# smileyenot983/reconstructor

Hardware: AMD Instinct MI355X
Metric: descriptor pair-distances/s + BA LM-iterations/s (1k cams, 100k pts) (higher is better)
Workload: dtype f16+f64

## Files before the change

reconstructor_amd/csrc/match.hip:

```cpp
#include "rcn_internal.h"

#include <algorithm>
#include <cmath>

typedef _Float16 half8 __attribute__((ext_vector_type(8)));
typedef float f32x16 __attribute__((ext_vector_type(16)));
typedef float f32x4 __attribute__((ext_vector_type(4)));
typedef unsigned u32x4 __attribute__((ext_vector_type(4)));

#define RCN_QT 512
#define RCN_GROUP 4
#define RCN_TBL_BYTES ((RCN_GROUP * 24 + 127) / 128 * 128)
#define RCN_NBUF 4
#define RCN_PD 2
#define RCN_CHUNK_ROWS (1ll << 27)
#define RCN_BT 64
#define RCN_PAD_HN 1.0e30f
#define RCN_I8_IDX_BITS 12
#define RCN_I8_IDX_MASK ((1u << RCN_I8_IDX_BITS) - 1u)
#define RCN_I8_PAD_ACC ((1 << (32 - RCN_I8_IDX_BITS)) - 1)
#define RCN_I8_BT 128
#define RCN_I8_RES_MAX 8.01
#define RCN_I8_M_MAX 720.0
#define RCN_I8_PEAK_MAX 8.0
// ... 635 lines not shown
        }
    } else {
        for (int k = 0; k < D; ++k) {
            double d = (double)q[k] - (double)t[k];
            acc = fma(d, d, acc);
        }
    }
    return acc;
}

__device__ __forceinline__ bool ratio_pass(double d2_best, double d2_second, float ratio)
{
    float dist0 = sqrtf((float)d2_best);
    float dist1 = sqrtf((float)d2_second);
    return dist0 < ratio * dist1;
}

struct RerankArgs {
    const ImgDev *imgs;
    const int32_t *pairs;
    const uint2 *cand;
    int32_t *out;
    int64_t out_stride;
    unsigned long long *fb_list;
    unsigned *fb_count;
    unsigned *fb_tacc;
    unsigned long long *sv_list;
    unsigned *sv_count;
    int32_t n_pairs, kq_stride, D, qblocks, pair_base;
    uint32_t idx_mask;
    float ratio;
    const ScaleDev *sc;
    int32_t all_to_fallback;
    int32_t filter_pass, rerank_pass;
};

#ifdef RCN_DIAG
#define RCN_FILTER_PASS(a) ((a).filter_pass != 0)
#define RCN_RERANK_PASS(a) ((a).rerank_pass != 0)
#else
#define RCN_FILTER_PASS(a) false
#define RCN_RERANK_PASS(a) false
#endif

__device__ __forceinline__ int certify(double ea, int ia, double eb, double lbnc, float ratio)
{
    const bool nn_certain = ea < lbnc;
    double lb1 = fmin(eb, lbnc), lb0 = fmin(ea, lbnc);
    if (lb1 < 0.0) lb1 = 0.0;
    if (lb0 < 0.0) lb0 = 0.0;
    if (nn_certain && ratio_pass(ea, lb1, ratio)) return ia;
    if (!ratio_pass(lb0, eb, ratio)) return -1;
    return -2;
}

__device__ __forceinline__ double coarse_eps(const ScaleDev &a, double nq2)
{
    const double nq = sqrt(nq2) * (1.0 + 1e-12);
    const double mag = a.s2 * nq * a.n_max;
    return a.c_in * nq * a.n_max + a.c_sub * (nq + a.n_max) + 1e-9 + a.c_acc * (a.hn_max + mag) +
           6.0e-8 * a.hn_max;
}
__device__ __forceinline__ double acc_to_d2(const ScaleDev &a, double nq2, double acc)
{
    return nq2 + (2.0 / a.s2) * (acc - a.bias);
}

__device__ __forceinline__ double key_lo(const ScaleDev &S, unsigned k, uint32_t mask)
{
    return S.coarse_i8 ? (double)(k >> RCN_I8_IDX_BITS) : (double)__uint_as_float(k & ~mask);
}
__device__ __forceinline__ double key_hi(const ScaleDev &S, unsigned k, uint32_t mask)
{
    return S.coarse_i8 ? (double)(k >> RCN_I8_IDX_BITS) : (double)__uint_as_float((k & ~mask) + mask + 1u);
}
__device__ __forceinline__ bool key_is_pad(const ScaleDev &S, unsigned k, uint32_t mask)
{
    return S.coarse_i8 ? (k >> RCN_I8_IDX_BITS) >= (unsigned)RCN_I8_PAD_ACC : !(__uint_as_float(k & ~mask) < 1.0e29f);
}
__device__ __forceinline__ int key_idx(const ScaleDev &S, unsigned k, uint32_t mask)
{
    return (int)(k & (S.coarse_i8 ? RCN_I8_IDX_MASK : mask));
}
__device__ __forceinline__ double coarse_eps_row(const ScaleDev &S, const ImgDev &qi, int q, double nq2)
{
    if (!S.coarse_i8) return coarse_eps(S, nq2);
    const float2 n = qi.i8n[q];
    return ((double)n.x * S.rho + (double)n.y * (S.tau + S.rho)) * (1.0 + 1e-9) + 0.5 + 1.0e-3;
}

__device__ __forceinline__ double big_lower_bound(const unsigned long long *bigmin, double nq2)
{
    const double b2 = __longlong_as_double((long long)*bigmin);
    if (!(b2 <= 1.7976931348623157e308)) return b2;
    const double d = sqrt(b2) * (1.0 - 1e-12) - sqrt(nq2) * (1.0 + 1e-12);
    return d > 0.0 ? d * d * (1.0 - 1e-9) : 0.0;
}

__device__ __forceinline__ unsigned mid_thr_acc(const ScaleDev &S, const ImgDev &qi, int q, double nq2, double eb, unsigned key2, uint32_t mask)
{
    if (!S.coarse_i8 || key_is_pad(S, key2, mask) || !(fabs(eb) <= 1.7976931348623157e308)) return 0u;
    const double d2 = eb * (1.0 + S.rel_slack) + S.rel_slack * (nq2 + S.n_max * S.n_max);
    const double v = floor(S.bias + S.hs2 * (d2 - nq2) + coarse_eps_row(S, qi, q, nq2)) + 1.0;
    if (!(v >= 1.0) || v >= (double)RCN_I8_PAD_ACC) return 0u;
    return (unsigned)v;
}

__device__ __forceinline__ void list_append(unsigned long long *list, unsigned *count, bool want,
                                            unsigned long long entry, unsigned *side = nullptr, unsigned side_value = 0u)
{
    const unsigned long long m = __ballot(want);
    if (!m) return;
    const int lane = threadIdx.x & 63;
    const int leader = __ffsll((long long)m) - 1;
    unsigned base = 0;
    if (lane == leader) base = atomicAdd(count, (unsigned)__popcll(m));
    base = __shfl(base, leader);
    if (want) {
        const unsigned slot = base + __popcll(m & ((1ull << lane) - 1ull));
        list[slot] = entry;
        if (side) side[slot] = side_value;
    }
}

#define RCN_FT 1024
#define RCN_FR 4
#define RCN_FB (RCN_FT * RCN_FR)
__global__ __launch_bounds__(RCN_FT) void k_filter(RerankArgs a)
{
    __shared__ unsigned wcnt[2][RCN_FT / 64];
    __shared__ unsigned wbase[2][RCN_FT / 64];
    const int pl = blockIdx.x / a.qblocks, pair = a.pair_base + pl;
    const int q0 = (blockIdx.x - pl * a.qblocks) * RCN_FB + threadIdx.x;
    const ScaleDev S = *a.sc;
    const ImgDev qi = a.imgs[a.pairs[2 * pair]];
    const ImgDev ti = a.imgs[a.pairs[2 * pair + 1]];
    unsigned survm = 0u, fbm = 0u;
    double nq2v[RCN_FR];
    uint2 cv[RCN_FR];
#pragma unroll
    for (int r = 0; r < RCN_FR; ++r) {
        const int q = q0 + r * RCN_FT;
        nq2v[r] = 0.0; cv[r] = make_uint2(0u, 0u);
        if (q < qi.K && ti.K >= 2) {
            nq2v[r] = qi.nrm2[q];
            if (!a.all_to_fallback) cv[r] = a.cand[(size_t)pair * a.kq_stride + q];
        }
    }
#pragma unroll
    for (int r = 0; r < RCN_FR; ++r) {
        const int q = q0 + r * RCN_FT;
        bool surv = false, fb = false;
        if (q < qi.K) {
            int32_t res = -1;
            if (ti.K >= 2) {
                const double nq2 = nq2v[r];
                const uint2 c = cv[r];
                if (a.all_to_fallback || !(nq2 < S.thr2)  || key_is_pad(S, c.y, a.idx_mask)) fb = true;
                else {
                    const double eps = coarse_eps_row(S, qi, q, nq2);
                    const double lb_big = big_lower_bound(ti.bigmin, nq2);
                    const double slack = S.rel_slack * (nq2 + S.n_max * S.n_max);
                    const double lo = key_lo(S, c.x, a.idx_mask);
                    const double hi = key_hi(S, c.y, a.idx_mask);
                    double lb0 = fmin(acc_to_d2(S, nq2, lo - eps) - slack, lb_big);
                    const double ub1 = acc_to_d2(S, nq2, hi + eps) + slack;
                    if (lb0 < 0.0) lb0 = 0.0;
                    surv = ratio_pass(lb0, ub1, a.ratio) || RCN_FILTER_PASS(a);
                    if (surv && ti.K > 2 && !RCN_FILTER_PASS(a)) {
                        const double hi0 = key_hi(S, c.x, a.idx_mask);
                        const double lo1 = key_lo(S, c.y, a.idx_mask);
                        const double ub0 = acc_to_d2(S, nq2, hi0 + eps) + slack;
                        double lbnc = fmin(acc_to_d2(S, nq2, lo1 - eps) - slack, lb_big);
                        if (lbnc < 0.0) lbnc = 0.0;
                        if (ub0 >= 0.0 && ub0 < lbnc && ratio_pass(ub0, lbnc, a.ratio)) {
                            res = (int32_t)key_idx(S, c.x, a.idx_mask);
                            surv = false;
                        }
                    }
                }
            }
            a.out[(size_t)pair * a.out_stride + q] = res;
        }
        survm |= surv ? 1u << r : 0u;
        fbm |= fb ? 1u << r : 0u;
    }
    const int lane = threadIdx.x & 63, w = threadIdx.x >> 6, nw = blockDim.x >> 6;
    unsigned ns = 0, nf = 0;
#pragma unroll
    for (int r = 0; r < RCN_FR; ++r) { ns += (unsigned)__popcll(__ballot(survm >> r & 1u)); nf += (unsigned)__popcll(__ballot(fbm >> r & 1u)); }
    if (lane == 0) { wcnt[0][w] = ns; wcnt[1][w] = nf; }
    __syncthreads();
    if (threadIdx.x < 2) {
        unsigned tot = 0;
        for (int i = 0; i < nw; ++i) { wbase[threadIdx.x][i] = tot; tot += wcnt[threadIdx.x][i]; }
        const unsigned base = tot ? atomicAdd(threadIdx.x == 0 ? a.sv_count : a.fb_count, tot) : 0u;
        for (int i = 0; i < nw; ++i) wbase[threadIdx.x][i] += base;
    }
    __syncthreads();
    const unsigned long long lt = (1ull << lane) - 1ull;
    unsigned bs = wbase[0][w], bf = wbase[1][w];
#pragma unroll
    for (int r = 0; r < RCN_FR; ++r) {
        const unsigned long long entry = ((unsigned long long)pair << 32) | (unsigned)(q0 + r * RCN_FT);
        const unsigned long long ms = __ballot(survm >> r & 1u), mf = __ballot(fbm >> r & 1u);
        if (survm >> r & 1u) a.sv_list[bs + __popcll(ms & lt)] = entry;
        if (fbm >> r & 1u) a.fb_list[bf + __popcll(mf & lt)] = entry;
        bs += (unsigned)__popcll(ms); bf += (unsigned)__popcll(mf);
    }
}

#define RR_ROWS 192
#define RR_LD 36
__global__ __launch_bounds__(64) void k_rerank_lds(RerankArgs a)
{
    __shared__ __attribute__((aligned(16))) float tile[RR_ROWS * RR_LD];
    __shared__ const float *rowptr[RR_ROWS];
    const int lane = threadIdx.x;
    const unsigned n = *a.sv_count;
    const int D = a.D;
    const int nchunk = (D + 31) / 32;
    const ScaleDev S = *a.sc;
    for (unsigned g = blockIdx.x; g * 64u < n; g += gridDim.x) {
        const unsigned sidx = g * 64u + lane;
        const bool live = sidx < n;
        const unsigned long long e = a.sv_list[live ? sidx : g * 64u];
        const int pair = (int)(e >> 32), q = (int)(e & 0xFFFFFFFFu);
        const ImgDev qi = a.imgs[a.pairs[2 * pair]];
        const ImgDev ti = a.imgs[a.pairs[2 * pair + 1]];
        const uint2 c = a.cand[(size_t)pair * a.kq_stride + q];
        int ia = key_idx(S, c.x, a.idx_mask), ib = key_idx(S, c.y, a.idx_mask);
        if (ib >= ti.K) ib = ia;
        __syncthreads();
        rowptr[lane] = qi.f32 + (size_t)q * D;
        rowptr[64 + lane] = ti.f32 + (size_t)ia * D;
        rowptr[128 + lane] = ti.f32 + (size_t)ib * D;
        __syncthreads();
        double acc = 0.0, acc2 = 0.0;
        const float *qrow = tile + lane * RR_LD;
        const float *trow = tile + (64 + lane) * RR_LD;
        const float *trow2 = tile + (128 + lane) * RR_LD;
        for (int ch = 0; ch < nchunk; ++ch) {
            const int col = ch * 32 + (lane & 7) * 4;
#pragma unroll
            for (int i = 0; i < RR_ROWS / 8; ++i) {
                const int r = i * 8 + (lane >> 3);
                float4 v = make_float4(0.f, 0.f, 0.f, 0.f);
                if (col < D) v = *reinterpret_cast<const float4 *>(rowptr[r] + col);
                *reinterpret_cast<float4 *>(tile + r * RR_LD + (lane & 7) * 4) = v;
            }
            __syncthreads();
            const int kmax = min(32, D - ch * 32);
            for (int k4 = 0; k4 < kmax; k4 += 4) {
                const float4 x = *reinterpret_cast<const float4 *>(qrow + k4);
                const float4 y = *reinterpret_cast<const float4 *>(trow + k4);
                const float4 z = *reinterpret_cast<const float4 *>(trow2 + k4);
                double d;
                d = (double)x.x - (double)y.x; acc = fma(d, d, acc);
                d = (double)x.y - (double)y.y; acc = fma(d, d, acc);
                d = (double)x.z - (double)y.z; acc = fma(d, d, acc);
                d = (double)x.w - (double)y.w; acc = fma(d, d, acc);
                d = (double)x.x - (double)z.x; acc2 = fma(d, d, acc2);
                d = (double)x.y - (double)z.y; acc2 = fma(d, d, acc2);
                d = (double)x.z - (double)z.z; acc2 = fma(d, d, acc2);
                d = (double)x.w - (double)z.w; acc2 = fma(d, d, acc2);
            }
            __syncthreads();
        }
        bool fb = false;
        unsigned tacc = 0u;
        if (live) {
            double ea = acc, eb = acc2;
            if (ib != ia && (eb < ea || (eb == ea && ib < ia))) { ea = acc2; eb = acc; const int t = ia; ia = ib; ib = t; }
            int res = -2;
            if (ti.K > 2 && ib != ia) {
                const double nq2 = qi.nrm2[q];
                const double lbacc = key_lo(S, c.y, a.idx_mask);
                const double lbnc = fmin(acc_to_d2(S, nq2, lbacc - coarse_eps_row(S, qi, q, nq2)) - S.rel_slack * (nq2 + S.n_max * S.n_max), big_lower_bound(ti.bigmin, nq2));
                res = RCN_RERANK_PASS(a) ? -2 : certify(ea, ia, eb, lbnc, a.ratio);
                if (res == -2 && a.fb_tacc) tacc = mid_thr_acc(S, qi, q, nq2, eb, c.y, a.idx_mask);
            }
            if (res >= 0) a.out[(size_t)pair * a.out_stride + q] = res;
            else if (res == -2) fb = true;
        }
        list_append(a.fb_list, a.fb_count, fb, e, a.fb_tacc, tacc);
    }
}

__global__ void k_rerank_generic(RerankArgs a)
{
    const unsigned n = *a.sv_count;
    const ScaleDev S = *a.sc;
    for (unsigned s = blockIdx.x * blockDim.x + threadIdx.x; s < n; s += gridDim.x * blockDim.x) {
        const unsigned long long e = a.sv_list[s];
        const int pair = (int)(e >> 32), q = (int)(e & 0xFFFFFFFFu);
        const ImgDev qi = a.imgs[a.pairs[2 * pair]];
        const ImgDev ti = a.imgs[a.pairs[2 * pair + 1]];
        const uint2 c = a.cand[(size_t)pair * a.kq_stride + q];
        int ia = key_idx(S, c.x, a.idx_mask), ib = key_idx(S, c.y, a.idx_mask);
        const float *qrow = qi.f32 + (size_t)q * a.D;
        double ea = exact_d2<false>(qrow, ti.f32 + (size_t)ia * a.D, a.D);
        double eb = exact_d2<false>(qrow, ti.f32 + (size_t)ib * a.D, a.D);
        if (eb < ea || (eb == ea && ib < ia)) { double te = ea; ea = eb; eb = te; ia = ib; }
        double lbnc = INFINITY;
        const double nq2 = qi.nrm2[q];
        if (ti.K > 2) {
            const double lbacc = key_lo(S, c.y, a.idx_mask);
            lbnc = fmin(acc_to_d2(S, nq2, lbacc - coarse_eps_row(S, qi, q, nq2)) - S.rel_slack * (nq2 + S.n_max * S.n_max), big_lower_bound(ti.bigmin, nq2));
        }
        int res = RCN_RERANK_PASS(a) ? -2 : certify(ea, ia, eb, lbnc, a.ratio);
        if (res == -2) {
            unsigned slot = atomicAdd(a.fb_count, 1u);
            a.fb_list[slot] = e;
            if (a.fb_tacc) a.fb_tacc[slot] = ti.K > 2 && ib != ia ? mid_thr_acc(S, qi, q, nq2, eb, c.y, a.idx_mask) : 0u;
            res = -1;
        }
        a.out[(size_t)pair * a.out_stride + q] = res;
    }
}

__device__ __forceinline__ void merge_top2(double &b0, int &i0, double &b1, int &i1, double c0, int j0, double c1, int j1)
{
    const bool mine = (b0 < c0) || (b0 == c0 && i0 < j0);
    const double f0 = mine ? b0 : c0; const int fi0 = mine ? i0 : j0;
    const double l0 = mine ? c0 : b0; const int li0 = mine ? j0 : i0;
    const double s0 = mine ? b1 : c1; const int si0 = mine ? i1 : j1;
    const bool pick = (l0 < s0) || (l0 == s0 && li0 < si0);
    b0 = f0; i0 = fi0;
    b1 = pick ? l0 : s0; i1 = pick ? li0 : si0;
}

template <bool VEC4>
__global__ __launch_bounds__(256) void k_exact_rows(const ImgDev *__restrict__ imgs,
                                                     const int32_t *__restrict__ pairs,
                                                     const unsigned long long *__restrict__ list,
                                                     const unsigned *__restrict__ count, int D,
                                                     float ratio, int32_t *__restrict__ out,
                                                     int64_t out_stride, unsigned skip = 0)
{
    __shared__ double sb[4][2];
    __shared__ int si[4][2];
    const int lane = threadIdx.x & 63, w = threadIdx.x >> 6;
    const unsigned n = *count;
    for (unsigned it = skip + blockIdx.x; it < n; it += gridDim.x) {
        const unsigned long long e = list[it];
        const int pair = (int)(e >> 32), q = (int)(e & 0xFFFFFFFFu);
        const ImgDev qi = imgs[pairs[2 * pair]];
        const ImgDev ti = imgs[pairs[2 * pair + 1]];
        const float *qrow = qi.f32 + (size_t)q * D;
        double b0 = INFINITY, b1 = INFINITY;
        int i0 = 0x7FFFFFFF, i1 = 0x7FFFFFFF;
        for (int j = threadIdx.x; j < ti.K; j += 256) {
            double d = exact_d2<VEC4>(qrow, ti.f32 + (size_t)j * D, D);
            if (d < b0) { b1 = b0; i1 = i0; b0 = d; i0 = j; }
            else if (d < b1) { b1 = d; i1 = j; }
        }
        for (int o = 32; o; o >>= 1) {
            const double c0 = __shfl_xor(b0, o), c1 = __shfl_xor(b1, o);
            const int j0 = __shfl_xor(i0, o), j1 = __shfl_xor(i1, o);
            merge_top2(b0, i0, b1, i1, c0, j0, c1, j1);
        }
        __syncthreads();
        if (lane == 0) { sb[w][0] = b0; sb[w][1] = b1; si[w][0] = i0; si[w][1] = i1; }
        __syncthreads();
        if (threadIdx.x == 0) {
            for (int k = 1; k < 4; ++k) merge_top2(b0, i0, b1, i1, sb[k][0], si[k][0], sb[k][1], si[k][1]);
            out[(size_t)pair * out_stride + q] = ratio_pass(b0, b1, ratio) ? i0 : -1;
        }
    }
// ... 323 lines not shown
                }
            }
        }
    }
}
__global__ __launch_bounds__(256, 4) void k_mid_eval(MidArgs a)
{
    __shared__ __attribute__((aligned(16))) float tt[256 * MID_LD];
    __shared__ __attribute__((aligned(16))) float tq[RCN_MIDQ * MID_LD];
    __shared__ const float *qptr[RCN_MIDQ];
    __shared__ float thr[RCN_MIDQ], qnorm[RCN_MIDQ];
    __shared__ float red[4][RCN_MIDQ][2];
    __shared__ unsigned qslot[RCN_MIDQ];
    __shared__ int s_need2, s_bin, s_nown;
    const int t = threadIdx.x, lane = t & 63, w = t >> 6;
    const unsigned n_items = *a.n_items;
    for (unsigned it = blockIdx.x; it < n_items; it += gridDim.x) {
        __syncthreads();
        if (t == 0) {
            int lo = 0, hi = a.n_slots;
            while (hi - lo > 1) { const int mid = (lo + hi) >> 1; if (a.ibase[mid] <= it) lo = mid; else hi = mid; }
            s_bin = lo;
            s_need2 = 0;
        }
        __syncthreads();
        const int bin = s_bin;
        const unsigned k = it - a.ibase[bin], h = a.offs[bin + 1] - a.offs[bin];
        const int first = (int)(a.offs[bin] + RCN_MIDQ * k), nall = (int)min((unsigned)RCN_MIDQ, h - RCN_MIDQ * k);
        const ImgDev ti = a.imgs[bin];
        if (t < 64) {
            const bool own = t < nall && a.tacc[first + t] == 0u;
            const unsigned long long om = __ballot(own);
            if (t == 0) s_nown = __popcll(om);
            if (own) {
                const int o = __popcll(om & ((1ull << t) - 1ull));
                const unsigned long long e = a.sorted[first + t];
                const int pair = (int)(e >> 32), q = (int)(e & 0xFFFFFFFFu);
                const ImgDev qi = a.imgs[a.pairs[2 * pair]];
                qslot[o] = (unsigned)(first + t);
                qptr[o] = qi.f32 + (size_t)q * a.D;
                qnorm[o] = (float)(sqrt(qi.nrm2[q]) * (1.0 + 1e-6));
                const float th = a.thr[first + t];
                thr[o] = th;
                if (!(th < INFINITY)) s_need2 = 1;
            }
        }
        __syncthreads();
        const int nq = s_nown;
        if (nq == 0) continue;
        float m1[RCN_MIDQ], m2[RCN_MIDQ];
        if (!s_need2) {
            mid_sweep<0>(a, ti, qptr, nq, qslot, thr, qnorm, ti.K, tt, tq, m1, m2);
            continue;
        }
        const int prefix = min(ti.K, max(512, ti.K / 4));
#pragma unroll
        for (int q = 0; q < RCN_MIDQ; ++q) { m1[q] = INFINITY; m2[q] = INFINITY; }
        mid_sweep<1>(a, ti, qptr, nq, qslot, thr, qnorm, prefix, tt, tq, m1, m2);
#pragma unroll
        for (int q = 0; q < RCN_MIDQ; ++q) {
            float b1 = m1[q], b2 = m2[q];
            for (int o = 32; o; o >>= 1) {
                const float c1 = __shfl_xor(b1, o), c2 = __shfl_xor(b2, o);
                const float lo = fminf(b1, c1), hi = fmaxf(b1, c1);
                b2 = fminf(hi, fminf(b2, c2)); b1 = lo;
            }
            if (lane == 0) { red[w][q][0] = b1; red[w][q][1] = b2; }
        }
        __syncthreads();
        if (t < nq) {
            float b1 = red[0][t][0], b2 = red[0][t][1];
            for (int kk = 1; kk < 4; ++kk) {
                const float c1 = red[kk][t][0], c2 = red[kk][t][1];
                const float lo = fminf(b1, c1), hi = fmaxf(b1, c1);
                b2 = fminf(hi, fminf(b2, c2)); b1 = lo;
            }
            thr[t] = b2 < INFINITY ? b2 + fabsf(b2) * 1.0e-6f : INFINITY;
        }
        __syncthreads();
        mid_sweep<2>(a, ti, qptr, nq, qslot, thr, qnorm, ti.K, tt, tq, m1, m2);
    }
}
#include "mid_i8.h"
__global__ __launch_bounds__(256) void k_mid_exact(MidArgs a)
{
    const unsigned n = mid_rows(a);
    const int lane = threadIdx.x & 63;
    for (unsigned r = blockIdx.x * 4 + (threadIdx.x >> 6); r < n; r += gridDim.x * 4) {
        const unsigned long long e = a.sorted[r];
        const int pair = (int)(e >> 32), q = (int)(e & 0xFFFFFFFFu);
        const unsigned cnt = a.ccount[r];
        if (cnt > (unsigned)RCN_MIDCAP) {
            if (lane == 0) a.fb2_list[atomicAdd(a.fb2_count, 1u)] = e;
            continue;
        }
        const ImgDev qi = a.imgs[a.pairs[2 * pair]];
        const ImgDev ti = a.imgs[a.pairs[2 * pair + 1]];
        double b0 = INFINITY, b1 = INFINITY;
        int i0 = 0x7FFFFFFF, i1 = 0x7FFFFFFF;
        if (lane < (int)cnt) {
            i0 = a.clist[(size_t)r * RCN_MIDCAP + lane];
            b0 = exact_d2<true>(qi.f32 + (size_t)q * a.D, ti.f32 + (size_t)i0 * a.D, a.D);
            if (!(b0 < INFINITY)) { b0 = INFINITY; i0 = 0x7FFFFFFF; }
        }
        for (int o = 32; o; o >>= 1) {
            const double c0 = __shfl_xor(b0, o), c1 = __shfl_xor(b1, o);
            const int j0 = __shfl_xor(i0, o), j1 = __shfl_xor(i1, o);
            merge_top2(b0, i0, b1, i1, c0, j0, c1, j1);
        }
        if (lane == 0) a.out[(size_t)pair * a.out_stride + q] = ratio_pass(b0, b1, a.ratio) ? i0 : -1;
    }
}

__global__ void k_unique_claim(const ImgDev *__restrict__ imgs, const int32_t *__restrict__ pairs,
                               const int32_t *__restrict__ out, int64_t out_stride,
                               int32_t *__restrict__ owner, int owner_stride, int qblocks, int pair_base)
{
    const int pl = blockIdx.x / qblocks, pair = pair_base + pl;
    const int q = (blockIdx.x - pl * qblocks) * blockDim.x + threadIdx.x;
    if (q >= imgs[pairs[2 * pair]].K) return;
    const int t = out[(size_t)pair * out_stride + q];
    if (t >= 0) atomicMin(owner + (size_t)pair * owner_stride + t, q);
}

__global__ void k_unique_emit(const ImgDev *__restrict__ imgs, const int32_t *__restrict__ pairs,
                              int32_t *__restrict__ out, int64_t out_stride,
                              const int32_t *__restrict__ owner, int owner_stride,
                              int32_t *__restrict__ counts, int qblocks, int pair_base)
{
    const int pl = blockIdx.x / qblocks, pair = pair_base + pl;
    const int q = (blockIdx.x - pl * qblocks) * blockDim.x + threadIdx.x;
    if (q >= out_stride) return;
    int32_t *o = out + (size_t)pair * out_stride + q;
    bool keep = false;
    if (q < imgs[pairs[2 * pair]].K) {
        const int t = *o;
        keep = t >= 0 && owner[(size_t)pair * owner_stride + t] == q;
    }
    if (!keep) *o = -1;
    const unsigned long long m = __ballot(keep);
    if ((threadIdx.x & 63) == 0 && m) atomicAdd(counts + pair, (int)__popcll(m));
}

#define RCN_UNIQ_LDS 8192
__global__ __launch_bounds__(256) void k_unique_pair(const ImgDev *__restrict__ imgs, const int32_t *__restrict__ pairs,
                                                     int32_t *__restrict__ out, int64_t out_stride,
                                                     int32_t *__restrict__ counts, int pair_base)
{
    __shared__ int owner[RCN_UNIQ_LDS];
    __shared__ int wsum[4];
    const int pair = pair_base + blockIdx.x, t = threadIdx.x;
    const int Kq = imgs[pairs[2 * pair]].K, Kt = imgs[pairs[2 * pair + 1]].K;
    for (int i = t; i < Kt; i += 256) owner[i] = 0x7fffffff;
    __syncthreads();
    int32_t *row = out + (size_t)pair * out_stride;
    for (int q = t; q < Kq; q += 256) {
        const int tr = row[q];
        if (tr >= 0) atomicMin(&owner[tr], q);
    }
    __syncthreads();
    int kept = 0;
    for (int q0 = 0; q0 < out_stride; q0 += 256) {
        const int q = q0 + t;
        bool keep = false;
        if (q < out_stride) {
            const int tr = q < Kq ? row[q] : -1;
            keep = tr >= 0 && owner[tr] == q;
            if (!keep && (q >= Kq || tr >= 0)) row[q] = -1;
        }
        kept += (int)__popcll(__ballot(keep));
    }
    if ((t & 63) == 0) wsum[t >> 6] = kept;
    __syncthreads();
    if (t == 0) counts[pair] = wsum[0] + wsum[1] + wsum[2] + wsum[3];
}

__global__ void k_stats_acc(unsigned *c, int mid, unsigned midrows)
{
    if (threadIdx.x != 0 || blockIdx.x != 0) return;
    c[4] += c[0];
    c[5] += c[1];
    c[6] += mid ? c[2] + (c[0] > midrows ? c[0] - midrows : 0u) : c[0];
}

static int pad_dim(int D)
{
    if (D <= 32) return 32;
    if (D <= 64) return 64;
    if (D <= 128) return 128;
    if (D <= 256) return 256;
    return 0;
}

static hipError_t launch_rowstats(rcn_ctx *ctx, const float *x, int rows, int D, double *nrm2, unsigned *cnt)
{
    ctx->hist_rows += rows;
    unsigned long long *mx = reinterpret_cast<unsigned long long *>(cnt + 2);
    if (D % 4 == 0 && (reinterpret_cast<uintptr_t>(x) & 15) == 0)
        k_rowstats<true><<<std::max(1, std::min((rows + 15) / 16, 4096)), 256, 0, ctx->stream>>>(x, rows, D, nrm2, cnt, mx, cnt + RCN_HIST_WORD);
    else
        k_rowstats<false><<<std::max(1, std::min((rows + 3) / 4, 4096)), 256, 0, ctx->stream>>>(x, rows, D, nrm2, cnt, mx, cnt + RCN_HIST_WORD);
    return hipGetLastError();
}

static void free_image(ImgHost &im)
{
    if (im.slab >= 0) return;
    if (im.f32) (void)hipFree(im.f32);
    if (im.f16) (void)hipFree(im.f16);
    if (im.hn) (void)hipFree(im.hn);
    if (im.nrm2) (void)hipFree(im.nrm2);
    if (im.bigmin) (void)hipFree(im.bigmin);
    if (im.i8n) (void)hipFree(im.i8n);
    im.f32 = nullptr; im.f16 = nullptr; im.hn = nullptr; im.nrm2 = nullptr; im.bigmin = nullptr; im.i8n = nullptr;
}

static void free_slab(Slab &sl)
{
    if (sl.f16) (void)hipFree(sl.f16);
    if (sl.hn) (void)hipFree(sl.hn);
    if (sl.nrm2) (void)hipFree(sl.nrm2);
    if (sl.bigmin) (void)hipFree(sl.bigmin);
    if (sl.i8n) (void)hipFree(sl.i8n);
    if (sl.own_f32) (void)hipFree(sl.own_f32);
    if (sl.own_Ks) (void)hipFree(sl.own_Ks);
    sl = Slab();
}

static void retire_unreferenced_slabs(rcn_ctx *ctx)
{
    std::vector<char> used(ctx->slabs.size(), 0);
    for (const auto &kv : ctx->images)
        if (kv.second.slab >= 0) used[kv.second.slab] = 1;
    for (size_t i = 0; i < ctx->slabs.size(); ++i)
        if (ctx->slabs[i].live && !used[i]) free_slab(ctx->slabs[i]);
}

int rcn_match_release(rcn_ctx *ctx)
{
    for (auto &kv : ctx->images) free_image(kv.second);
    ctx->images.clear();
    for (Slab &sl : ctx->slabs) free_slab(sl);
    ctx->slabs.clear();
    ctx->table_host.clear();
    ctx->prepared = false;
    ctx->D = ctx->DP = 0;
    return RCN_OK;
}

static int ensure_counters(rcn_ctx *ctx)
{
    if (!ctx->counters.p) {
        RCN_HIP(ctx->counters.reserve(RCN_COUNTER_BYTES));
        RCN_HIP(hipMemsetAsync(ctx->counters.p, 0, RCN_COUNTER_BYTES, ctx->stream));
    }
    return RCN_OK;
}

static int drop_scratch_if_alone(rcn_ctx *ctx, int32_t D)
{
    if (ctx->images.empty() || ctx->D == D) return RCN_OK;
    for (const auto &kv : ctx->images)
        if (kv.first != INT32_MIN && kv.first != INT32_MIN + 1) return RCN_OK;
    RCN_HIP(hipStreamSynchronize(ctx->stream));
    for (auto &kv : ctx->images) free_image(kv.second);
    ctx->images.clear();
    ctx->prepared = false;
    return RCN_OK;
}

static int upload_common(rcn_ctx *ctx, int32_t img_id, const float *src, bool src_is_device,
                         int32_t K, int32_t D)
{
    if (!ctx || K < 0 || D <= 0 || (K > 0 && !src)) {
// ... 582 lines not shown
        if (mfma) {
            CoarseArgs ca;
            ca.imgs = imgs; ca.pairs = pairs; ca.cand = cand_c;
            const int ng_c = chunk_ng[c];
            ca.groups = ctx->groups_dev.as<int2>() + chunk_off[c];
            ca.n_groups = ng_c; ca.tiles_per_pair = tiles; ca.kq_stride = kq_stride;
            const int64_t items = (int64_t)ng_c * tiles;
            ca.items_per_xcd = (int)((items + 7) / 8);
            ca.idx_mask = idx_mask;
            ca.sc = ctx->scale_dev.as<ScaleDev>();
            const int blocks = ca.items_per_xcd * 8;
            hipError_t e;
            if (ctx->coarse_w4 && ctx->DP >= 64) {
                switch (ctx->DP) {
                case 64: e = launch_coarse_w4<64>(ctx, ca, blocks); break;
                case 128: e = launch_coarse_w4<128>(ctx, ca, blocks); break;
                default: e = launch_coarse_w4<256>(ctx, ca, blocks); break;
                }
            } else {
                const int shape = ctx->coarse_shape >= 0 ? ctx->coarse_shape : (ctx->DP == 256 ? 1 : 0);
                if (shape == 1) {
                    switch (ctx->DP) {
                    case 32: e = launch_coarse<32, 0, 1>(ctx, ca, blocks); break;
                    case 64: e = launch_coarse<64, 0, 1>(ctx, ca, blocks); break;
                    case 128: e = launch_coarse<128, 0, 1>(ctx, ca, blocks); break;
                    default:
#ifdef RCN_DIAG
                        switch (ctx->ablate) {
                        case 1: e = launch_coarse<256, 1, 1>(ctx, ca, blocks); break;
                        case 9: e = launch_coarse<256, 9, 1>(ctx, ca, blocks); break;
                        default: e = launch_coarse<256, 0, 1>(ctx, ca, blocks); break;
                        }
#else
                        e = launch_coarse<256, 0, 1>(ctx, ca, blocks);
#endif
                        break;
                    }
                } else {
                    switch (ctx->DP) {
                    case 32:
#ifdef RCN_DIAG
                        if (ctx->ablate == 1) { e = launch_coarse<32, 1, 0>(ctx, ca, blocks); break; }
                        if (ctx->ablate == 2) { e = launch_coarse<32, 2, 0>(ctx, ca, blocks); break; }
                        if (ctx->ablate == 6) { e = launch_coarse<32, 6, 0>(ctx, ca, blocks); break; }
#endif
                        e = launch_coarse<32>(ctx, ca, blocks); break;
                    case 64: e = launch_coarse<64>(ctx, ca, blocks); break;
                    case 128:
#ifdef RCN_DIAG
                        if (ctx->ablate == 1) { e = launch_coarse<128, 1, 0>(ctx, ca, blocks); break; }
                        if (ctx->ablate == 2) { e = launch_coarse<128, 2, 0>(ctx, ca, blocks); break; }
                        if (ctx->ablate == 6) { e = launch_coarse<128, 6, 0>(ctx, ca, blocks); break; }
#endif
                        e = launch_coarse<128>(ctx, ca, blocks); break;
                    default: e = launch_coarse<256>(ctx, ca, blocks); break;
                    }
                }
            }
            RCN_HIP(e);
            if (ctx->i8_allowed) {
#ifdef RCN_DIAG
                if (ctx->coarse_i8_shape == 0) e = launch_coarse_i8<0, 0>(ctx, ca, blocks);
                else if (ctx->ablate == 1) e = launch_coarse_i8<1, 1>(ctx, ca, blocks);
                else
#endif
                e = launch_coarse_i8<0, 1>(ctx, ca, blocks);
                RCN_HIP(e);
            }
        }
        if (tm) RCN_HIP(hipEventRecord(ctx->ev_c[evi][c][1], st));
        ra.cand = cand_c;
        ra.pair_base = p0;
        ra.fb_list = ctx->fb_list.as<unsigned long long>(); ra.fb_count = ccnt;
        ra.sv_list = ctx->sv_list.as<unsigned long long>(); ra.sv_count = ccnt + 1;
        if (c > 0) RCN_HIP(hipMemsetAsync(ccnt, 0, 4 * sizeof(unsigned), st));
        if (kq_max > 0) {
            const int qblocks = (kq_max + 255) / 256;
            dim3 g((unsigned)qblocks * (unsigned)np_c);
            ra.qblocks = (kq_max + RCN_FB - 1) / RCN_FB;
            k_filter<<<(unsigned)ra.qblocks * (unsigned)np_c, RCN_FT, 0, st>>>(ra);
            RCN_HIP(hipGetLastError());
            if (ctx->f32_ready) RCN_HIP(hipStreamWaitEvent(st, ctx->f32_ready, 0));
            if (mfma) {
                if (vec4) k_rerank_lds<<<ctx->prop.multiProcessorCount * 16, 64, 0, st>>>(ra);
                else k_rerank_generic<<<ctx->prop.multiProcessorCount * 8, 256, 0, st>>>(ra);
                RCN_HIP(hipGetLastError());
            }
            const int fb_blocks = ctx->prop.multiProcessorCount * 8;
            const unsigned long long *brute = ra.fb_list;
            const unsigned *brute_n = ccnt;
            if (mid) {
                char *mw = ctx->mid_ws.as<char>();
                MidArgs ma;
                memset(&ma, 0, sizeof(ma));
                ma.imgs = imgs; ma.pairs = pairs; ma.cand = cand_c; ma.fb_list = ra.fb_list; ma.fb_count = ccnt; ma.tacc_in = ra.fb_tacc;
                if (defer) {
                    MidArgs md = ma;
                    md.sc = ra.sc; md.kq_stride = kq_stride; md.D = ctx->D; md.all_to_fallback = ra.all_to_fallback; md.idx_mask = idx_mask;
                    k_mid_defer<<<ctx->prop.multiProcessorCount * 2, 256, 0, st>>>(md, (unsigned long long *)(mw + mo_def), (float *)(mw + mo_defthr), (unsigned *)(mw + mo_deftacc), ccnt, (unsigned)mid_rows_cap);
                    k_mid_defer_commit<<<1, 64, 0, st>>>(ccnt, (unsigned)mid_rows_cap);
                }
                ma.sorted = (unsigned long long *)(mw + mo_sorted); ma.thr = (float *)(mw + mo_thr); ma.ccount = (unsigned *)(mw + mo_cc); ma.tacc = (unsigned *)(mw + mo_tacc);
                ma.clist = (int32_t *)(mw + mo_cl); ma.fb2_list = (unsigned long long *)(mw + mo_fb2);
                ma.hist = (unsigned *)(mw + mo_bins); ma.offs = ma.hist + (n_slots + 1); ma.cursor = ma.offs + (n_slots + 1); ma.ibase = ma.cursor + (n_slots + 1);
                ma.n_items = ccnt + 3; ma.fb2_count = ccnt + 2;
                ma.out = out_dev; ma.out_stride = out_stride; ma.sc = ra.sc; ma.n_slots = n_slots; ma.kq_stride = kq_stride; ma.D = ctx->D;
                ma.all_to_fallback = ra.all_to_fallback; ma.idx_mask = idx_mask; ma.ratio = ratio; ma.midrows = (uint32_t)ctx->mid_rows;
                const int mb = ctx->prop.multiProcessorCount * 4;
                k_mid_hist<<<mb, 256, 0, st>>>(ma);
                k_mid_bins<<<1, 1024, 0, st>>>(ma);
                k_mid_scatter<<<mb, 256, 0, st>>>(ma);
                k_mid_eval<<<ctx->prop.multiProcessorCount * 4, 256, 0, st>>>(ma);
                if (mid_i8) k_mid_eval_i8<<<mid_i8_grid, 256, 0, st>>>(ma);
                k_mid_exact<<<mb, 256, 0, st>>>(ma);
                RCN_HIP(hipGetLastError());
                if (vec4) k_exact_rows_lds<<<fb_blocks, 64 * EX_WAVES, 0, st>>>(imgs, pairs, ma.fb2_list, ma.fb2_count, ctx->D, ratio, out_dev, out_stride);
                RCN_HIP(hipGetLastError());
                if (cap_rows > ctx->mid_rows) k_exact_rows_lds<<<fb_blocks, 64 * EX_WAVES, 0, st>>>(imgs, pairs, brute, brute_n, ctx->D, ratio, out_dev, out_stride, (unsigned)ctx->mid_rows);
            } else if (vec4) k_exact_rows_lds<<<fb_blocks, 64 * EX_WAVES, 0, st>>>(imgs, pairs, brute, brute_n, ctx->D, ratio, out_dev, out_stride);
            else k_exact_rows<false><<<fb_blocks, 256, 0, st>>>(imgs, pairs, brute, brute_n, ctx->D, ratio, out_dev, out_stride);
            RCN_HIP(hipGetLastError());
            k_stats_acc<<<1, 64, 0, st>>>(ccnt, mid ? 1 : 0, (unsigned)ctx->mid_rows);
            if (tm) RCN_HIP(hipEventRecord(ctx->ev_c[evi][c][2], st));
            if (!uniq_lds) k_unique_claim<<<g, 256, 0, st>>>(imgs, pairs, out_dev, out_stride, ctx->owner.as<int32_t>(), owner_stride, qblocks, p0);
            RCN_HIP(hipGetLastError());
        }
        if (defer) {  }
        else if (uniq_lds) k_unique_pair<<<np_c, 256, 0, st>>>(imgs, pairs, out_dev, out_stride, counts_dev, p0);
        else {
            const int eblocks = (int)((out_stride + 255) / 256);
            dim3 g((unsigned)eblocks * (unsigned)np_c);
            k_unique_emit<<<g, 256, 0, st>>>(imgs, pairs, out_dev, out_stride, ctx->owner.as<int32_t>(), owner_stride, counts_dev, eblocks, p0);
        }
        RCN_HIP(hipGetLastError());
        if (tm) RCN_HIP(hipEventRecord(ctx->ev_c[evi][c][kq_max > 0 ? 3 : 2], st));
        if (tm && kq_max <= 0) RCN_HIP(hipEventRecord(ctx->ev_c[evi][c][3], st));
    }
    ctx->ev_tail_on[evi] = false;
    if (defer) {
        if (prof) { RCN_HIP(hipEventRecord(ctx->ev_tail[evi][0], st)); ctx->ev_tail_on[evi] = true; }
        char *mw = ctx->mid_ws.as<char>();
        RCN_HIP(hipMemsetAsync(ccnt + 2, 0, 2 * sizeof(unsigned), st));
        MidArgs ma;
        memset(&ma, 0, sizeof(ma));
        ma.imgs = imgs; ma.pairs = pairs; ma.cand = nullptr; ma.fb_list = (const unsigned long long *)(mw + mo_def); ma.fb_count = ccnt + 7;
        ma.thr_in = (const float *)(mw + mo_defthr);
        ma.tacc_in = mid_i8 ? (const unsigned *)(mw + mo_deftacc) : nullptr;
        ma.sorted = (unsigned long long *)(mw + mo_sorted); ma.thr = (float *)(mw + mo_thr); ma.ccount = (unsigned *)(mw + mo_cc); ma.tacc = (unsigned *)(mw + mo_tacc);
        ma.clist = (int32_t *)(mw + mo_cl); ma.fb2_list = (unsigned long long *)(mw + mo_fb2);
        ma.hist = (unsigned *)(mw + mo_bins); ma.offs = ma.hist + (n_slots + 1); ma.cursor = ma.offs + (n_slots + 1); ma.ibase = ma.cursor + (n_slots + 1);
        ma.n_items = ccnt + 3; ma.fb2_count = ccnt + 2;
        ma.out = out_dev; ma.out_stride = out_stride; ma.sc = ra.sc; ma.n_slots = n_slots; ma.kq_stride = kq_stride; ma.D = ctx->D;
        ma.all_to_fallback = ra.all_to_fallback; ma.idx_mask = idx_mask; ma.ratio = ratio; ma.midrows = (uint32_t)mid_rows_cap;
        const int mb = ctx->prop.multiProcessorCount * 4;
        k_mid_hist<<<mb, 256, 0, st>>>(ma);
        k_mid_bins<<<1, 1024, 0, st>>>(ma);
        k_mid_scatter<<<mb, 256, 0, st>>>(ma);
        k_mid_eval<<<ctx->prop.multiProcessorCount * 4, 256, 0, st>>>(ma);
        if (mid_i8) k_mid_eval_i8<<<mid_i8_grid, 256, 0, st>>>(ma);
        k_mid_exact<<<mb, 256, 0, st>>>(ma);
        k_exact_rows_lds<<<ctx->prop.multiProcessorCount * 8, 64 * EX_WAVES, 0, st>>>(imgs, pairs, ma.fb2_list, ma.fb2_count, ctx->D, ratio, out_dev, out_stride);
        k_stats_acc_deferred<<<1, 64, 0, st>>>(ccnt);
        RCN_HIP(hipGetLastError());
        if (prof) RCN_HIP(hipEventRecord(ctx->ev_tail[evi][1], st));
        k_unique_pair<<<n_pairs, 256, 0, st>>>(imgs, pairs, out_dev, out_stride, counts_dev, 0);
        RCN_HIP(hipGetLastError());
        if (prof) RCN_HIP(hipEventRecord(ctx->ev_tail[evi][2], st));
    }
    if (prof) ctx->ev_n++;
    ctx->last_chunks = n_chunks;
    ctx->last_kq_stride = kq_stride; ctx->last_idx_mask = idx_mask; ctx->last_n_pairs = n_pairs;
    ctx->last_stats.rows_total = rows;
    ctx->last_stats.pair_distances = pd;
    ctx->last_stats.used_mfma_path = mfma ? 1 : 0;
    ctx->last_stats.coarse_dtype = mfma ? -1 : 0;
    ctx->last_stats.rows_exact_fallback = -1;
    ctx->last_stats.err_bound_d2 = -1.0;
    return RCN_OK;
}

extern "C" {

int rcn_desc_upload(rcn_ctx *ctx, int32_t img_id, const float *desc_host, int32_t K, int32_t D)
{
    if (!ctx) return RCN_ERR_ARG;
    std::lock_guard<std::mutex> lk(ctx->mu);
    return upload_common(ctx, img_id, desc_host, false, K, D);
}

int rcn_desc_upload_device(rcn_ctx *ctx, int32_t img_id, const float *desc_dev, int32_t K, int32_t D)
{
    if (!ctx) return RCN_ERR_ARG;
    std::lock_guard<std::mutex> lk(ctx->mu);
    return upload_common(ctx, img_id, desc_dev, true, K, D);
}

int rcn_desc_upload_batch_device(rcn_ctx *ctx, int32_t first_img_id, int32_t n_images,
                                 const float *desc_dev, int32_t K, int32_t D)
{
    if (!ctx) return RCN_ERR_ARG;
    std::lock_guard<std::mutex> lk(ctx->mu);
    return upload_batch(ctx, first_img_id, n_images, desc_dev, K, D);
}

int rcn_desc_upload_batch(rcn_ctx *ctx, int32_t first_img_id, int32_t n_images, const float *const *rows_host,
                          const int32_t *K, int32_t D)
{
    if (!ctx) return RCN_ERR_ARG;
    std::lock_guard<std::mutex> lk(ctx->mu);
    return upload_batch_host(ctx, first_img_id, n_images, rows_host, K, D);
}

int rcn_desc_remove(rcn_ctx *ctx, int32_t img_id)
{
    if (!ctx) return RCN_ERR_ARG;
    std::lock_guard<std::mutex> lk(ctx->mu);
    auto it = ctx->images.find(img_id);
    if (it == ctx->images.end()) return RCN_OK;
    RCN_HIP(hipSetDevice(ctx->device));
    RCN_HIP(hipStreamSynchronize(ctx->stream));
    free_image(it->second);
    ctx->images.erase(it);
    retire_unreferenced_slabs(ctx);
    ctx->prepared = false;
    if (ctx->images.empty()) ctx->D = ctx->DP = 0;
    return RCN_OK;
}

int rcn_desc_clear(rcn_ctx *ctx)
{
    if (!ctx) return RCN_ERR_ARG;
    std::lock_guard<std::mutex> lk(ctx->mu);
    RCN_HIP(hipSetDevice(ctx->device));
    RCN_HIP(hipStreamSynchronize(ctx->stream));
    rcn_match_release(ctx);
    if (ctx->counters.p) RCN_HIP(hipMemsetAsync(ctx->counters.p, 0, RCN_COUNTER_BYTES, ctx->stream));
    ctx->hist_rows = 0;
    return RCN_OK;
}

int rcn_desc_count(const rcn_ctx *ctx)
{
    if (!ctx) return 0;
// ... 271 lines not shown
```

Baseline: 4638 billion.

## Rework rerank and mid-exact kernels around a shared register-prefetched full-row LDS gather

Adds a common gather helper that loads up to 24 whole descriptor rows per wave into registers, then stores them into an XOR-swizzled LDS tile. The rerank kernel now processes 8 survivors per iteration and prefetches the next tile's rows and metadata while computing the current one. Fallback-list appends are buffered in shared memory and flushed in batches instead of using one atomic per wave per step. The mid-exact stage gets a new single-wave kernel that packs 4 query rows and 20 candidate rows per tile, and the old 256-thread kernel is kept for D above 256. Grid sizes now come from an occupancy query. The cost is fewer rows per wave, which may reduce parallelism, and higher register pressure from the 24 float4 prefetch registers.

Result: faster. 4725 billion, median of 6 (+1.9%).

```diff
diff --git a/reconstructor_amd/csrc/exact_gather.h b/reconstructor_amd/csrc/exact_gather.h
--- /dev/null
+++ b/reconstructor_amd/csrc/exact_gather.h
@@ -0,0 +1,79 @@
+#pragma once
+
+#define XG_ROWS 24
+#define XG_ROWF 256
+#define XG_TILEF (XG_ROWS * XG_ROWF)
+
+__device__ __forceinline__ unsigned xg_issue(float4 (&v)[XG_ROWS], const float *ptr, int D)
+{
+    const int col = (threadIdx.x & 63) * 4;
+    const unsigned long long pv = reinterpret_cast<unsigned long long>(ptr);
+    const int lo = (int)(unsigned)pv, hi = (int)(unsigned)(pv >> 32);
+#pragma unroll
+    for (int i = 0; i < XG_ROWS; ++i) {
+        const unsigned long long p = ((unsigned long long)(unsigned)__builtin_amdgcn_readlane(hi, i) << 32) | (unsigned)__builtin_amdgcn_readlane(lo, i);
+        v[i] = make_float4(0.f, 0.f, 0.f, 0.f);
+        if (p && col < D) v[i] = *reinterpret_cast<const float4 *>(reinterpret_cast<const float *>(p) + col);
+    }
+    return (unsigned)__ballot(ptr != nullptr) & ((1u << XG_ROWS) - 1u);
+}
+
+__device__ __forceinline__ void xg_store(float *tile, const float4 (&v)[XG_ROWS], unsigned rows)
+{
+    const int lane = threadIdx.x & 63;
+#pragma unroll
+    for (int i = 0; i < XG_ROWS; ++i)
+        if (rows >> i & 1u) *reinterpret_cast<float4 *>(tile + i * XG_ROWF + ((lane ^ (i & 15)) << 2)) = v[i];
+}
+
+__device__ __forceinline__ double xg_chain(const float *tile, int xr, int yr, int D)
+{
+    const float *x = tile + xr * XG_ROWF, *y = tile + yr * XG_ROWF;
+    const int sx = xr & 15, sy = yr & 15;
+    double acc = 0.0;
+#pragma unroll 4
+    for (int c = 0; c < D / 4; ++c) {
+        const float4 a = *reinterpret_cast<const float4 *>(x + ((c ^ sx) << 2));
+        const float4 b = *reinterpret_cast<const float4 *>(y + ((c ^ sy) << 2));
+        double d;
+        d = (double)a.x - (double)b.x; acc = fma(d, d, acc);
+        d = (double)a.y - (double)b.y; acc = fma(d, d, acc);
+        d = (double)a.z - (double)b.z; acc = fma(d, d, acc);
+        d = (double)a.w - (double)b.w; acc = fma(d, d, acc);
+    }
+    return acc;
+}
+
+#define XG_PEND 64
+#define XG_PEND_FLUSH (XG_PEND - XG_ROWS)
+struct XgPend {
+    unsigned long long e[XG_PEND];
+    unsigned side[XG_PEND];
+};
+__device__ __forceinline__ void xg_pend_flush(XgPend &p, unsigned &np, unsigned long long *list, unsigned *count, unsigned *side)
+{
+    if (!np) return;
+    const int lane = threadIdx.x & 63;
+    unsigned base = 0;
+    if (lane == 0) base = atomicAdd(count, np);
+    base = __builtin_amdgcn_readfirstlane(base);
+    if ((unsigned)lane < np) {
+        list[base + lane] = p.e[lane];
+        if (side) side[base + lane] = p.side[lane];
+    }
+    np = 0;
+}
+__device__ __forceinline__ void xg_pend_add(XgPend &p, unsigned &np, bool want, unsigned long long entry, unsigned side_value,
+                                            unsigned long long *list, unsigned *count, unsigned *side)
+{
+    const unsigned long long m = __ballot(want);
+    if (!m) return;
+    const int lane = threadIdx.x & 63;
+    if (want) {
+        const unsigned slot = np + __popcll(m & ((1ull << lane) - 1ull));
+        p.e[slot] = entry;
+        p.side[slot] = side_value;
+    }
+    np += (unsigned)__popcll(m);
+    if (np > XG_PEND_FLUSH) xg_pend_flush(p, np, list, count, side);
+}
diff --git a/reconstructor_amd/csrc/match.hip b/reconstructor_amd/csrc/match.hip
--- a/reconstructor_amd/csrc/match.hip
+++ b/reconstructor_amd/csrc/match.hip
@@ -741,28 +741,38 @@
 {
     return (int)(k & (S.coarse_i8 ? RCN_I8_IDX_MASK : mask));
 }
+__device__ __forceinline__ double coarse_eps_i8n(const ScaleDev &S, float2 n, double nq2)
+{
+    if (!S.coarse_i8) return coarse_eps(S, nq2);
+    return ((double)n.x * S.rho + (double)n.y * (S.tau + S.rho)) * (1.0 + 1e-9) + 0.5 + 1.0e-3;
+}
 __device__ __forceinline__ double coarse_eps_row(const ScaleDev &S, const ImgDev &qi, int q, double nq2)
 {
     if (!S.coarse_i8) return coarse_eps(S, nq2);
-    const float2 n = qi.i8n[q];
-    return ((double)n.x * S.rho + (double)n.y * (S.tau + S.rho)) * (1.0 + 1e-9) + 0.5 + 1.0e-3;
-}
-
-__device__ __forceinline__ double big_lower_bound(const unsigned long long *bigmin, double nq2)
-{
-    const double b2 = __longlong_as_double((long long)*bigmin);
+    return coarse_eps_i8n(S, qi.i8n[q], nq2);
+}
+
+__device__ __forceinline__ double big_lower_bound_bits(unsigned long long bigmin_bits, double nq2)
+{
+    const double b2 = __longlong_as_double((long long)bigmin_bits);
     if (!(b2 <= 1.7976931348623157e308)) return b2;
     const double d = sqrt(b2) * (1.0 - 1e-12) - sqrt(nq2) * (1.0 + 1e-12);
     return d > 0.0 ? d * d * (1.0 - 1e-9) : 0.0;
 }
-
-__device__ __forceinline__ unsigned mid_thr_acc(const ScaleDev &S, const ImgDev &qi, int q, double nq2, double eb, unsigned key2, uint32_t mask)
+__device__ __forceinline__ double big_lower_bound(const unsigned long long *bigmin, double nq2) { return big_lower_bound_bits(*bigmin, nq2); }
+
+__device__ __forceinline__ unsigned mid_thr_acc_eps(const ScaleDev &S, double eps, double nq2, double eb, unsigned key2, uint32_t mask)
 {
     if (!S.coarse_i8 || key_is_pad(S, key2, mask) || !(fabs(eb) <= 1.7976931348623157e308)) return 0u;
     const double d2 = eb * (1.0 + S.rel_slack) + S.rel_slack * (nq2 + S.n_max * S.n_max);
-    const double v = floor(S.bias + S.hs2 * (d2 - nq2) + coarse_eps_row(S, qi, q, nq2)) + 1.0;
+    const double v = floor(S.bias + S.hs2 * (d2 - nq2) + eps) + 1.0;
     if (!(v >= 1.0) || v >= (double)RCN_I8_PAD_ACC) return 0u;
     return (unsigned)v;
+}
+__device__ __forceinline__ unsigned mid_thr_acc(const ScaleDev &S, const ImgDev &qi, int q, double nq2, double eb, unsigned key2, uint32_t mask)
+{
+    if (!S.coarse_i8) return 0u;
+    return mid_thr_acc_eps(S, coarse_eps_row(S, qi, q, nq2), nq2, eb, key2, mask);
 }
 
 __device__ __forceinline__ void list_append(unsigned long long *list, unsigned *count, bool want,
@@ -869,81 +879,90 @@
     }
 }
 
-#define RR_ROWS 192
-#define RR_LD 36
+#include "exact_gather.h"
+#define RR_B (XG_ROWS / 3)
+struct RrRows {
+    unsigned long long e;
+    uint2 c;
+    const float *ptr;
+    double nq2;
+    float2 i8n;
+    unsigned long long bigmin;
+    int32_t ia, ib, tK;
+};
+__device__ __forceinline__ RrRows rr_rows(const RerankArgs &a, const ScaleDev &S, unsigned g, unsigned n)
+{
+    RrRows m;
+    const int lane = threadIdx.x & 63;
+    const unsigned sidx = g * RR_B + (lane % RR_B);
+    const bool live = sidx < n && lane < XG_ROWS;
+    m.e = a.sv_list[live ? sidx : g * RR_B];
+    const int pair = (int)(m.e >> 32), q = (int)(m.e & 0xFFFFFFFFu);
+    const ImgDev &qi = a.imgs[a.pairs[2 * pair]], &ti = a.imgs[a.pairs[2 * pair + 1]];
+    m.c = a.cand[(size_t)pair * a.kq_stride + q];
+    const float *qf = qi.f32, *tf = ti.f32;
+    m.tK = ti.K;
+    m.ia = key_idx(S, m.c.x, a.idx_mask); m.ib = key_idx(S, m.c.y, a.idx_mask);
+    if (m.ib >= m.tK) m.ib = m.ia;
+    const int role = lane / RR_B;
+    m.ptr = !live ? nullptr : role == 0 ? qf + (size_t)q * a.D : tf + (size_t)(role == 1 ? m.ia : m.ib) * a.D;
+    m.nq2 = 0.0; m.i8n = make_float2(0.f, 0.f); m.bigmin = 0ull;
+    if (live && role == 0 && m.tK > 2 && m.ib != m.ia) {
+        m.nq2 = qi.nrm2[q];
+        if (S.coarse_i8) m.i8n = qi.i8n[q];
+        m.bigmin = *ti.bigmin;
+    }
+    return m;
+}
 __global__ __launch_bounds__(64) void k_rerank_lds(RerankArgs a)
 {
-    __shared__ __attribute__((aligned(16))) float tile[RR_ROWS * RR_LD];
-    __shared__ const float *rowptr[RR_ROWS];
+    __shared__ __attribute__((aligned(16))) float tile[XG_TILEF];
+    __shared__ XgPend pend;
     const int lane = threadIdx.x;
     const unsigned n = *a.sv_count;
+    const unsigned ntile = (n + RR_B - 1) / RR_B;
     const int D = a.D;
-    const int nchunk = (D + 31) / 32;
     const ScaleDev S = *a.sc;
-    for (unsigned g = blockIdx.x; g * 64u < n; g += gridDim.x) {
-        const unsigned sidx = g * 64u + lane;
-        const bool live = sidx < n;
-        const unsigned long long e = a.sv_list[live ? sidx : g * 64u];
-        const int pair = (int)(e >> 32), q = (int)(e & 0xFFFFFFFFu);
-        const ImgDev qi = a.imgs[a.pairs[2 * pair]];
-        const ImgDev ti = a.imgs[a.pairs[2 * pair + 1]];
-        const uint2 c = a.cand[(size_t)pair * a.kq_stride + q];
-        int ia = key_idx(S, c.x, a.idx_mask), ib = key_idx(S, c.y, a.idx_mask);
-        if (ib >= ti.K) ib = ia;
-        __syncthreads();
-        rowptr[lane] = qi.f32 + (size_t)q * D;
-        rowptr[64 + lane] = ti.f32 + (size_t)ia * D;
-        rowptr[128 + lane] = ti.f32 + (size_t)ib * D;
-        __syncthreads();
-        double acc = 0.0, acc2 = 0.0;
-        const float *qrow = tile + lane * RR_LD;
-        const float *trow = tile + (64 + lane) * RR_LD;
-        const float *trow2 = tile + (128 + lane) * RR_LD;
-        for (int ch = 0; ch < nchunk; ++ch) {
-            const int col = ch * 32 + (lane & 7) * 4;
-#pragma unroll
-            for (int i = 0; i < RR_ROWS / 8; ++i) {
-                const int r = i * 8 + (lane >> 3);
-                float4 v = make_float4(0.f, 0.f, 0.f, 0.f);
-                if (col < D) v = *reinterpret_cast<const float4 *>(rowptr[r] + col);
-                *reinterpret_cast<float4 *>(tile + r * RR_LD + (lane & 7) * 4) = v;
-            }
-            __syncthreads();
-            const int kmax = min(32, D - ch * 32);
-            for (int k4 = 0; k4 < kmax; k4 += 4) {
-                const float4 x = *reinterpret_cast<const float4 *>(qrow + k4);
-                const float4 y = *reinterpret_cast<const float4 *>(trow + k4);
-                const float4 z = *reinterpret_cast<const float4 *>(trow2 + k4);
-                double d;
-                d = (double)x.x - (double)y.x; acc = fma(d, d, acc);
-                d = (double)x.y - (double)y.y; acc = fma(d, d, acc);
-                d = (double)x.z - (double)y.z; acc = fma(d, d, acc);
-                d = (double)x.w - (double)y.w; acc = fma(d, d, acc);
-                d = (double)x.x - (double)z.x; acc2 = fma(d, d, acc2);
-                d = (double)x.y - (double)z.y; acc2 = fma(d, d, acc2);
-                d = (double)x.z - (double)z.z; acc2 = fma(d, d, acc2);
-                d = (double)x.w - (double)z.w; acc2 = fma(d, d, acc2);
-            }
-            __syncthreads();
-        }
+    unsigned g = blockIdx.x, np = 0;
+    if (g >= ntile) return;
+    float4 v[XG_ROWS];
+    RrRows m0 = rr_rows(a, S, g, n), m1 = m0;
+    unsigned rows = xg_issue(v, m0.ptr, D);
+    if (g + gridDim.x < ntile) m1 = rr_rows(a, S, g + gridDim.x, n);
+    xg_store(tile, v, rows);
+    for (; g < ntile; g += gridDim.x) {
+        const bool more = g + gridDim.x < ntile;
+        if (more) rows = xg_issue(v, m1.ptr, D);
+        __builtin_amdgcn_wave_barrier();
+        double acc = 0.0;
+        if (lane < 2 * RR_B) acc = xg_chain(tile, lane % RR_B, RR_B + lane, D);
+        const double acc2 = __shfl(acc, lane + RR_B);
         bool fb = false;
         unsigned tacc = 0u;
-        if (live) {
+        if (lane < RR_B && g * RR_B + lane < n) {
+            const int pair = (int)(m0.e >> 32), q = (int)(m0.e & 0xFFFFFFFFu);
+            const uint2 c = m0.c;
+            int ia = m0.ia, ib = m0.ib;
             double ea = acc, eb = acc2;
             if (ib != ia && (eb < ea || (eb == ea && ib < ia))) { ea = acc2; eb = acc; const int t = ia; ia = ib; ib = t; }
             int res = -2;
-            if (ti.K > 2 && ib != ia) {
-                const double nq2 = qi.nrm2[q];
+            if (m0.tK > 2 && ib != ia) {
+                const double nq2 = m0.nq2, eps = coarse_eps_i8n(S, m0.i8n, nq2);
                 const double lbacc = key_lo(S, c.y, a.idx_mask);
-                const double lbnc = fmin(acc_to_d2(S, nq2, lbacc - coarse_eps_row(S, qi, q, nq2)) - S.rel_slack * (nq2 + S.n_max * S.n_max), big_lower_bound(ti.bigmin, nq2));
+                const double lbnc = fmin(acc_to_d2(S, nq2, lbacc - eps) - S.rel_slack * (nq2 + S.n_max * S.n_max), big_lower_bound_bits(m0.bigmin, nq2));
                 res = RCN_RERANK_PASS(a) ? -2 : certify(ea, ia, eb, lbnc, a.ratio);
-                if (res == -2 && a.fb_tacc) tacc = mid_thr_acc(S, qi, q, nq2, eb, c.y, a.idx_mask);
+                if (res == -2 && a.fb_tacc) tacc = mid_thr_acc_eps(S, eps, nq2, eb, c.y, a.idx_mask);
             }
             if (res >= 0) a.out[(size_t)pair * a.out_stride + q] = res;
             else if (res == -2) fb = true;
         }
-        list_append(a.fb_list, a.fb_count, fb, e, a.fb_tacc, tacc);
-    }
+        xg_pend_add(pend, np, fb, m0.e, tacc, a.fb_list, a.fb_count, a.fb_tacc);
+        m0 = m1;
+        if (g + 2 * gridDim.x < ntile) m1 = rr_rows(a, S, g + 2 * gridDim.x, n);
+        __builtin_amdgcn_wave_barrier();
+        if (more) xg_store(tile, v, rows);
+    }
+    xg_pend_flush(pend, np, a.fb_list, a.fb_count, a.fb_tacc);
 }
 
 __global__ void k_rerank_generic(RerankArgs a)
@@ -1433,7 +1452,90 @@
     }
 }
 #include "mid_i8.h"
-__global__ __launch_bounds__(256) void k_mid_exact(MidArgs a)
+#define MX_Q 4
+#define MX_C (XG_ROWS - MX_Q)
+__global__ __launch_bounds__(64) void k_mid_exact(MidArgs a)
+{
+    __shared__ __attribute__((aligned(16))) float tile[XG_TILEF];
+    __shared__ double sd[MX_C];
+    __shared__ int sj[MX_C];
+    const int lane = threadIdx.x;
+    const unsigned n = mid_rows(a);
+    const unsigned ngroup = (n + MX_Q - 1) / MX_Q;
+    const int D = a.D;
+    float4 v[XG_ROWS];
+    for (unsigned g = blockIdx.x; g < ngroup; g += gridDim.x) {
+        const unsigned r = g * MX_Q + lane;
+        const bool own = lane < MX_Q && r < n;
+        unsigned long long e = 0ull;
+        unsigned cnt = 0u;
+        unsigned long long qp = 0ull, tf = 0ull;
+        bool decide = false;
+        if (own) {
+            e = a.sorted[r];
+            cnt = a.ccount[r];
+            if (cnt > (unsigned)RCN_MIDCAP) {
+                a.fb2_list[atomicAdd(a.fb2_count, 1u)] = e;
+                cnt = 0u;
+            } else {
+                const int pair = (int)(e >> 32), q = (int)(e & 0xFFFFFFFFu);
+                qp = reinterpret_cast<unsigned long long>(a.imgs[a.pairs[2 * pair]].f32 + (size_t)q * D);
+                tf = reinterpret_cast<unsigned long long>(a.imgs[a.pairs[2 * pair + 1]].f32);
+                decide = true;
+            }
+        }
+        unsigned pre[MX_Q + 1], mine = 0u;
+        pre[0] = 0u;
+#pragma unroll
+        for (int t = 0; t < MX_Q; ++t) {
+            pre[t + 1] = pre[t] + (unsigned)__shfl((int)cnt, t);
+            if (lane > t) mine = pre[t + 1];
+        }
+        const unsigned total = pre[MX_Q];
+        double b0 = INFINITY, b1 = INFINITY;
+        int i0 = 0x7FFFFFFF, i1 = 0x7FFFFFFF;
+        for (unsigned base = 0; base < total; base += MX_C) {
+            const unsigned j = base + lane;
+            const bool cl = lane < MX_C && j < total;
+            int t = 0;
+            unsigned pt = 0u;
+#pragma unroll
+            for (int tt = 1; tt < MX_Q; ++tt)
+                if (j >= pre[tt]) { t = tt; pt = pre[tt]; }
+            const unsigned long long tft = __shfl(tf, t);
+            int idx = 0x7FFFFFFF;
+            unsigned long long cp = 0ull;
+            if (cl) {
+                idx = a.clist[(size_t)(g * MX_Q + t) * RCN_MIDCAP + (j - pt)];
+                cp = reinterpret_cast<unsigned long long>(reinterpret_cast<const float *>(tft) + (size_t)idx * D);
+            }
+            const unsigned long long cps = __shfl(cp, lane - MX_Q);
+            const unsigned long long ptr = lane < MX_Q ? (base == 0 ? qp : 0ull) : lane < XG_ROWS ? cps : 0ull;
+            const unsigned rows = xg_issue(v, reinterpret_cast<const float *>(ptr), D);
+            xg_store(tile, v, rows);
+            __builtin_amdgcn_wave_barrier();
+            double d = INFINITY;
+            if (cl) d = xg_chain(tile, t, MX_Q + lane, D);
+            if (lane < MX_C) { sd[lane] = d; sj[lane] = idx; }
+            __builtin_amdgcn_wave_barrier();
+            if (decide) {
+                const unsigned lo = max(mine, base), hi = min(mine + cnt, base + MX_C);
+                for (unsigned jj = lo; jj < hi; ++jj) {
+                    const double c0 = sd[jj - base];
+                    if (c0 < INFINITY)
+                        merge_top2(b0, i0, b1, i1, c0, sj[jj - base], INFINITY, 0x7FFFFFFF);
+                }
+            }
+            __builtin_amdgcn_wave_barrier();
+        }
+        if (decide) {
+            const int pair = (int)(e >> 32), q = (int)(e & 0xFFFFFFFFu);
+            a.out[(size_t)pair * a.out_stride + q] = ratio_pass(b0, b1, a.ratio) ? i0 : -1;
+        }
+    }
+}
+
+__global__ __launch_bounds__(256) void k_mid_exact_wide(MidArgs a)
 {
     const unsigned n = mid_rows(a);
     const int lane = threadIdx.x & 63;
@@ -1541,6 +1643,24 @@
     if (D <= 128) return 128;
     if (D <= 256) return 256;
     return 0;
+}
+
+template <typename Kernel>
+static int resident_grid(rcn_ctx *ctx, Kernel kernel, int &per_cu)
+{
+    if (per_cu <= 0) {
+        int nb = 0;
+        if (hipOccupancyMaxActiveBlocksPerMultiprocessor(&nb, kernel, 64, 0) != hipSuccess || nb < 1) nb = 4;
+        per_cu = nb;
+    }
+    return ctx->prop.multiProcessorCount * per_cu;
+}
+static int rerank_grid(rcn_ctx *ctx) { static int per_cu = 0; return resident_grid(ctx, k_rerank_lds, per_cu); }
+static void launch_mid_exact(rcn_ctx *ctx, const MidArgs &ma, hipStream_t st)
+{
+    static int per_cu = 0;
+    if (ma.D <= XG_ROWF) k_mid_exact<<<resident_grid(ctx, k_mid_exact, per_cu), 64, 0, st>>>(ma);
+    else k_mid_exact_wide<<<ctx->prop.multiProcessorCount * 4, 256, 0, st>>>(ma);
 }
 
 static hipError_t launch_rowstats(rcn_ctx *ctx, const float *x, int rows, int D, double *nrm2, unsigned *cnt)
@@ -2289,7 +2409,7 @@
             RCN_HIP(hipGetLastError());
             if (ctx->f32_ready) RCN_HIP(hipStreamWaitEvent(st, ctx->f32_ready, 0));
             if (mfma) {
-                if (vec4) k_rerank_lds<<<ctx->prop.multiProcessorCount * 16, 64, 0, st>>>(ra);
+                if (vec4) k_rerank_lds<<<rerank_grid(ctx), 64, 0, st>>>(ra);
                 else k_rerank_generic<<<ctx->prop.multiProcessorCount * 8, 256, 0, st>>>(ra);
                 RCN_HIP(hipGetLastError());
             }
@@ -2319,7 +2439,7 @@
                 k_mid_scatter<<<mb, 256, 0, st>>>(ma);
                 k_mid_eval<<<ctx->prop.multiProcessorCount * 4, 256, 0, st>>>(ma);
                 if (mid_i8) k_mid_eval_i8<<<mid_i8_grid, 256, 0, st>>>(ma);
-                k_mid_exact<<<mb, 256, 0, st>>>(ma);
+                launch_mid_exact(ctx, ma, st);
                 RCN_HIP(hipGetLastError());
                 if (vec4) k_exact_rows_lds<<<fb_blocks, 64 * EX_WAVES, 0, st>>>(imgs, pairs, ma.fb2_list, ma.fb2_count, ctx->D, ratio, out_dev, out_stride);
                 RCN_HIP(hipGetLastError());
@@ -2365,7 +2485,7 @@
         k_mid_scatter<<<mb, 256, 0, st>>>(ma);
         k_mid_eval<<<ctx->prop.multiProcessorCount * 4, 256, 0, st>>>(ma);
         if (mid_i8) k_mid_eval_i8<<<mid_i8_grid, 256, 0, st>>>(ma);
-        k_mid_exact<<<mb, 256, 0, st>>>(ma);
+        launch_mid_exact(ctx, ma, st);
         k_exact_rows_lds<<<ctx->prop.multiProcessorCount * 8, 64 * EX_WAVES, 0, st>>>(imgs, pairs, ma.fb2_list, ma.fb2_count, ctx->D, ratio, out_dev, out_stride);
         k_stats_acc_deferred<<<1, 64, 0, st>>>(ccnt);
         RCN_HIP(hipGetLastError());
```
